# zhaodong-liu/GRAM

Hardware: AMD Instinct MI355X
Metric: users/sec @ beam=20 top-20 gen, Beauty T5-base; Recall@5 parity (higher is better)
Workload: dtype f16x3

## Files before the change

gram_amd/csrc/dec_attn.hip:

```cpp
#include <type_traits>

#include "common.h"
#include "prof.h"
#include "xattn_tile.h"

namespace {

__device__ __forceinline__ void xa_merge_w(float m0, float m1, float l0, float l1, float& w0, float& w1, float& inv) {
  const float M = fmaxf(fmaxf(GRAM_FMIN, m0), m1);
  w0 = __expf(m0 - M);
  w1 = __expf(m1 - M);
  inv = 1.f / __builtin_fmaf(l1, w1, l0 * w0);
}
__device__ __forceinline__ f32x4 xa_merge_o(f32x4 o0, f32x4 o1, float w0, float w1, float inv) {
  f32x4 r;
#pragma unroll
  for (int e = 0; e < 4; ++e) r[e] = __builtin_fmaf(o1[e], w1, o0[e] * w0) * inv;
  return r;
}

template <int NT, bool LIVE, int S, int NW>
__global__ __launch_bounds__(NW * 64) void cross_attn_kernel(
    const p16* __restrict__ q, const p16* __restrict__ kbank, const p16* __restrict__ vtbank,
    const uint8_t* __restrict__ mask, p16* __restrict__ out, int K, int H, int Sk, const int32_t* __restrict__ users,
    const int32_t* __restrict__ rowpos, long q_pstride, long bank_pstride, const uint32_t* __restrict__ key_bits) {
  using T = SplitTab<S>;
  constexpr int NB = NT * 16;
  static_assert(NW == 1 || NW == 2, "the merge is written for two waves");
  constexpr int PSTR = 2 * XA_TILE;
  constexpr int STAGE = S * PSTR;
  extern __shared__ __attribute__((aligned(16))) char smem[];
  float* sm_m = reinterpret_cast<float*>(smem);
  float* sm_l = sm_m + NW * NB;
  float* sm_o = sm_l + NW * NB;

  const int h = blockIdx.x, b = LIVE ? users[blockIdx.y] : blockIdx.y;
  const int tid = threadIdx.x, lane = tid & 63;
  const int wave = __builtin_amdgcn_readfirstlane(tid >> 6);
  const int c = lane & 15, g = lane >> 4;
  const int inner = H * 64;
  const char* kb = reinterpret_cast<const char*>(kbank + ((size_t)b * H + h) * Sk * 64);
  const char* vt = reinterpret_cast<const char*>(vtbank + ((size_t)b * H + h) * 64 * Sk);
  const uint8_t* mk = mask + (size_t)b * Sk;

  p16x8 qf[S][NT][2];
  f32x4 o[4][NT];
  float m[NT], l[NT];
#pragma unroll
  for (int nt = 0; nt < NT; ++nt) {
    m[nt] = GRAM_FMIN;
    l[nt] = 0.f;
#pragma unroll
    for (int mt = 0; mt < 4; ++mt) o[mt][nt] = (f32x4){0.f, 0.f, 0.f, 0.f};
  }

#pragma unroll
  for (int nt = 0; nt < NT; ++nt) {
    const int qrow = xa_row<LIVE>(b, K, 16 * nt + c, rowpos);
#pragma unroll
    for (int pc = 0; pc < S; ++pc)
#pragma unroll
      for (int kd = 0; kd < 2; ++kd)
        qf[pc][nt][kd] = qrow >= 0 ? ld_global_b128(q + pc * q_pstride + (size_t)qrow * inner + h * 64 + 32 * kd + 8 * g) : zero_bf16x8();
  }
  const int nsteps = Sk >> 5;
  uint32_t kb0 = 0, kb1 = 0;
  if (key_bits) {
    if (lane < nsteps) kb0 = key_bits[(size_t)b * 128 + lane];
    if (lane + 64 < nsteps) kb1 = key_bits[(size_t)b * 128 + 64 + lane];
  } else {
#pragma unroll
    for (int half = 0; half < 2; ++half) {
      const int st = lane + 64 * half;
      uint32_t bits = 0;
      if (st < nsteps) {
        const uint4* p = reinterpret_cast<const uint4*>(mk + 32 * st);
        const uint4 a = p[0], c2 = p[1];
        const uint32_t w8[8] = {a.x, a.y, a.z, a.w, c2.x, c2.y, c2.z, c2.w};
#pragma unroll
        for (int i = 0; i < 8; ++i)
#pragma unroll
          for (int j = 0; j < 4; ++j) bits |= ((w8[i] >> (8 * j)) & 0xffu) ? (1u << (4 * i + j)) : 0u;
      }
      if (half == 0) kb0 = bits; else kb1 = bits;
    }
  }
  unsigned long long v0 = __ballot(kb0 != 0u), v1 = __ballot(kb1 != 0u);
  if ((v0 | v1) == 0ull) {
    v0 = nsteps >= 64 ? ~0ull : ((1ull << nsteps) - 1ull);
    v1 = nsteps > 64 ? ((nsteps >= 128 ? ~0ull : ((1ull << (nsteps - 64)) - 1ull))) : 0ull;
  }
  v0 = __builtin_amdgcn_readfirstlane((unsigned)v0) | ((unsigned long long)__builtin_amdgcn_readfirstlane((unsigned)(v0 >> 32)) << 32);
  v1 = __builtin_amdgcn_readfirstlane((unsigned)v1) | ((unsigned long long)__builtin_amdgcn_readfirstlane((unsigned)(v1 >> 32)) << 32);
  int ord = 0;
  auto next = [&](int s) -> int {
    for (s = s + 1; s < nsteps; ++s) {
      const unsigned long long bit = (s < 64 ? (v0 >> s) : (v1 >> (s - 64))) & 1ull;
      if (bit) {
        const bool mine = ord == wave;
        ord = ord + 1 == NW ? 0 : ord + 1;
        if (mine) return s;
      }
    }
    return nsteps;
  };

  uint32_t koff[4], voff[4];
#pragma unroll
  for (int i = 0; i < 4; ++i) {
    const int kr = 8 * i + (lane >> 3);
    koff[i] = (uint32_t)(kr * 128 + (((lane & 7) ^ ksw(kr)) << 4));
    const int d = 16 * i + (lane >> 2);
    voff[i] = (uint32_t)(d * 64 + (((lane & 3) ^ vsw(d)) << 4));
  }
  const uint32_t stage0 = (uint32_t)(uintptr_t)(__attribute__((address_space(3))) char*)smem + wave * STAGE;
  auto issue_k = [&](int step) {
    const uint32_t dst = stage0;
#pragma unroll
    for (int pc = 0; pc < S; ++pc) {
      const char* kbase = kb + (size_t)pc * bank_pstride * 2 + (size_t)step * (32 * 128);
#pragma unroll
      for (int i = 0; i < 4; ++i) dma16_nt(dst + pc * PSTR + i * 1024, koff[i], kbase);
    }
  };
  auto issue_v = [&](int step) {
    const uint32_t dst = stage0;
#pragma unroll
    for (int pc = 0; pc < S; ++pc) {
      const char* vbase = vt + (size_t)pc * bank_pstride * 2 + (size_t)step * 4096;
#pragma unroll
      for (int i = 0; i < 4; ++i) dma16(dst + pc * PSTR + XA_TILE + i * 1024, voff[i], vbase);
    }
  };
  const int krow = 8 * (c >> 2) + (c & 3);
  p16x8 kf[S][2][2], vf[S][4];
  auto read_k = [&]() {
    const char* stg = smem + wave * STAGE;
#pragma unroll
    for (int pc = 0; pc < S; ++pc)
#pragma unroll
      for (int t = 0; t < 2; ++t)
#pragma unroll
        for (int kd = 0; kd < 2; ++kd) {
          const int r = krow + 4 * t;
          kf[pc][t][kd] = *reinterpret_cast<const p16x8*>(stg + pc * PSTR + r * 128 + (((g + 4 * kd) ^ ksw(r)) << 4));
        }
  };
  auto read_v = [&]() {
    const char* stg = smem + wave * STAGE;
#pragma unroll
    for (int pc = 0; pc < S; ++pc)
#pragma unroll
      for (int mt = 0; mt < 4; ++mt) {
        const int d = 16 * mt + c;
        vf[pc][mt] = *reinterpret_cast<const p16x8*>(stg + pc * PSTR + XA_TILE + d * 64 + ((g ^ vsw(d)) << 4));
      }
  };
  p16x8 pf[S][NT];
  auto math_qk = [&](int step) {
    const uint32_t kword = step < 64 ? (uint32_t)__builtin_amdgcn_readlane((int)kb0, step) : (uint32_t)__builtin_amdgcn_readlane((int)kb1, step - 64);
    const uint32_t kbits = kword >> (8 * g);
#pragma unroll
    for (int nt = 0; nt < NT; ++nt) {
      f32x4 s[2];
#pragma unroll
      for (int t = 0; t < 2; ++t) {
        f32x4 a = (f32x4){0.f, 0.f, 0.f, 0.f};
#pragma unroll
        for (int pr = 0; pr < T::NP; ++pr) {
          a = mfma16(kf[T::A[pr]][t][0], qf[T::B[pr]][nt][0], a);
          a = mfma16(kf[T::A[pr]][t][1], qf[T::B[pr]][nt][1], a);
        }
#pragma unroll
        for (int j = 0; j < 4; ++j) a[j] = ((kbits >> (4 * t + j)) & 1u) ? a[j] : GRAM_FMIN;
        s[t] = a;
      }
      float tm = fmaxf(fmaxf(fmaxf(s[0][0], s[0][1]), fmaxf(s[0][2], s[0][3])),
                       fmaxf(fmaxf(s[1][0], s[1][1]), fmaxf(s[1][2], s[1][3])));
      tm = fmaxf(tm, __shfl_xor(tm, 16, 64));
      tm = fmaxf(tm, __shfl_xor(tm, 32, 64));
      const float mn = fmaxf(m[nt], tm);
      const float alpha = __expf(m[nt] - mn);
      m[nt] = mn;
      float ps = 0.f;
#pragma unroll
      for (int t = 0; t < 2; ++t)
#pragma unroll
        for (int j = 0; j < 4; ++j) {
          float e = __expf(s[t][j] - mn);
          ps += e;
#pragma unroll
          for (int pc = 0; pc < S; ++pc) {
            const p16 eb = (p16)e;
            pf[pc][nt][4 * t + j] = eb;
            e -= (float)eb;
          }
        }
      l[nt] = xa_l_update(l[nt], alpha, ps);
#pragma unroll
      for (int mt = 0; mt < 4; ++mt) o[mt][nt] *= alpha;
    }
  };
  auto math_pv = [&]() {
#pragma unroll
    for (int mt = 0; mt < 4; ++mt)
#pragma unroll
      for (int nt = 0; nt < NT; ++nt)
#pragma unroll
        for (int pr = 0; pr < T::NP; ++pr) o[mt][nt] = mfma16(vf[T::A[pr]][mt], pf[T::B[pr]][nt], o[mt][nt]);
  };

  wait_vm<0>();
#pragma unroll
  for (int nt = 0; nt < NT; ++nt)
#pragma unroll
    for (int pc = 0; pc < S; ++pc)
#pragma unroll
      for (int kd = 0; kd < 2; ++kd) asm volatile("" : "+v"(qf[pc][nt][kd]));
  int cur = next(-1);
  if (cur < nsteps) {
    issue_k(cur);
    issue_v(cur);
  }
  while (cur < nsteps) {
    const int nxt = next(cur);
    wait_vm<4 * S>();
    read_k();
    if (nxt < nsteps) {
      asm volatile("s_waitcnt lgkmcnt(0)" ::: "memory");
      issue_k(nxt);
    }
    math_qk(cur);
    if (nxt < nsteps) wait_vm<4 * S>();
    else wait_vm<0>();
    read_v();
    if (nxt < nsteps) {
      asm volatile("s_waitcnt lgkmcnt(0)" ::: "memory");
      issue_v(nxt);
    }
    math_pv();
    cur = nxt;
  }

  if constexpr (NW == 1) {
#pragma unroll
    for (int nt = 0; nt < NT; ++nt) {
      float lt = l[nt];
      lt += __shfl_xor(lt, 16, 64);
      lt += __shfl_xor(lt, 32, 64);
      const float inv = 1.f / lt;
      const int orow = xa_row<LIVE>(b, K, 16 * nt + c, rowpos);
      if (orow >= 0) {
#pragma unroll
        for (int mt = 0; mt < 4; ++mt) xa_store<S>(out, orow, inner, h * 64 + 16 * mt + 4 * g, o[mt][nt] * inv);
      }
    }
    return;
  }
  gram_sync();
#pragma unroll
  for (int nt = 0; nt < NT; ++nt) {
    float lt = l[nt];
    lt += __shfl_xor(lt, 16, 64);
    lt += __shfl_xor(lt, 32, 64);
    const int beam = 16 * nt + c;
    if (g == 0) {
      sm_m[wave * NB + beam] = m[nt];
      sm_l[wave * NB + beam] = lt;
    }
#pragma unroll
    for (int mt = 0; mt < 4; ++mt)
      *reinterpret_cast<f32x4*>(sm_o + ((size_t)(wave * NB + beam)) * 64 + 16 * mt + 4 * g) = o[mt][nt];
  }
  gram_sync();
  for (int idx = tid; idx < K * 16; idx += NW * 64) {
    const int beam = idx >> 4, d4 = (idx & 15) * 4;
    float w0, w1, inv2;
    xa_merge_w(sm_m[beam], sm_m[NB + beam], sm_l[beam], sm_l[NB + beam], w0, w1, inv2);
    const f32x4 v = xa_merge_o(*reinterpret_cast<const f32x4*>(sm_o + ((size_t)beam) * 64 + d4),
                         *reinterpret_cast<const f32x4*>(sm_o + ((size_t)(NB + beam)) * 64 + d4), w0, w1, inv2);
    int orow = b * K + beam;
    if constexpr (LIVE) orow = rowpos[orow];
    if (orow >= 0) xa_store<S>(out, orow, inner, h * 64 + d4, v);
  }
}

constexpr int XA_RUN_MERGE = 4 * (4 * 64 * 16 + 2 * 64 * 4);
template <int S, int NW>
__global__ __launch_bounds__(2 * NW * 64, 2) void cross_attn_runs_kernel(
    const p16* __restrict__ q, const p16* __restrict__ kbank, const p16* __restrict__ vtbank, const uint8_t* __restrict__ mask,
    p16* __restrict__ out, int n_entries, int H, int Sk, const int32_t* __restrict__ ent_users, const int32_t* __restrict__ ent_rows,
    long q_pstride, long bank_pstride, const uint32_t* __restrict__ key_bits) {
  using T = SplitTab<S>;
  static_assert(NW == 1 || NW == 2, "the merge is written for two waves");
  constexpr int ER = GRAM_TAIL_ENTRY_ROWS;
  constexpr int MT = 4;
  static_assert(ER == 64, "a pair of entries is eight 16-row tiles");
  constexpr int PSTR = 2 * XA_TILE;
  constexpr int STAGE = S * PSTR;
  constexpr int MERGE = XA_RUN_MERGE;
  static_assert(MERGE == MT * (4 * 64 * 16 + 2 * 64 * 4), "O, m, l of up to MT tiles, one slot per lane");
  extern __shared__ __attribute__((aligned(16))) char smem[];

  const int h = blockIdx.x, lead = blockIdx.y;
  const int b = ent_users[lead];
  if (lead > 0 && ent_users[lead - 1] == b) return;
  int run_end = lead + 1;
  while (run_end < n_entries && ent_users[run_end] == b) ++run_end;

  const int tid = threadIdx.x, lane = tid & 63;
  const int wv = __builtin_amdgcn_readfirstlane(tid >> 6);
  const int wave = wv % NW, half = wv / NW;
  const int c = lane & 15, g = lane >> 4;
  const int inner = H * 64;
  const char* kb = reinterpret_cast<const char*>(kbank + ((size_t)b * H + h) * Sk * 64);
  const char* vt = reinterpret_cast<const char*>(vtbank + ((size_t)b * H + h) * 64 * Sk);
  const uint8_t* mk = mask + (size_t)b * Sk;

  const int nsteps = Sk >> 5;
  uint32_t kb0 = 0, kb1 = 0;
  if (key_bits) {
    if (lane < nsteps) kb0 = key_bits[(size_t)b * 128 + lane];
    if (lane + 64 < nsteps) kb1 = key_bits[(size_t)b * 128 + 64 + lane];
  } else {
#pragma unroll
    for (int hf = 0; hf < 2; ++hf) {
      const int st = lane + 64 * hf;
      uint32_t bits = 0;
      if (st < nsteps) {
        const uint4* p = reinterpret_cast<const uint4*>(mk + 32 * st);
        const uint4 a = p[0], c2 = p[1];
        const uint32_t w8[8] = {a.x, a.y, a.z, a.w, c2.x, c2.y, c2.z, c2.w};
#pragma unroll
        for (int i = 0; i < 8; ++i)
#pragma unroll
          for (int j = 0; j < 4; ++j) bits |= ((w8[i] >> (8 * j)) & 0xffu) ? (1u << (4 * i + j)) : 0u;
      }
      if (hf == 0) kb0 = bits; else kb1 = bits;
    }
  }
  unsigned long long v0 = __ballot(kb0 != 0u), v1 = __ballot(kb1 != 0u);
  if ((v0 | v1) == 0ull) {
    v0 = nsteps >= 64 ? ~0ull : ((1ull << nsteps) - 1ull);
    v1 = nsteps > 64 ? ((nsteps >= 128 ? ~0ull : ((1ull << (nsteps - 64)) - 1ull))) : 0ull;
  }
  v0 = __builtin_amdgcn_readfirstlane((unsigned)v0) | ((unsigned long long)__builtin_amdgcn_readfirstlane((unsigned)(v0 >> 32)) << 32);
  v1 = __builtin_amdgcn_readfirstlane((unsigned)v1) | ((unsigned long long)__builtin_amdgcn_readfirstlane((unsigned)(v1 >> 32)) << 32);
  int ord = 0;
  auto next = [&](int s) -> int {
    for (s = s + 1; s < nsteps; ++s) {
      const unsigned long long bit = (s < 64 ? (v0 >> s) : (v1 >> (s - 64))) & 1ull;
      if (bit) {
        const bool mine = ord == wave;
        ord = ord + 1 == NW ? 0 : ord + 1;
        if (mine) return s;
      }
    }
    return nsteps;
  };

  uint32_t koff[4], voff[4];
#pragma unroll
  for (int i = 0; i < 4; ++i) {
    const int kr = 8 * i + (lane >> 3);
    koff[i] = (uint32_t)(kr * 128 + (((lane & 7) ^ ksw(kr)) << 4));
    const int d = 16 * i + (lane >> 2);
    voff[i] = (uint32_t)(d * 64 + (((lane & 3) ^ vsw(d)) << 4));
  }
  const uint32_t stage0 = (uint32_t)(uintptr_t)(__attribute__((address_space(3))) char*)smem + wave * 2 * STAGE;
  const int nvalid = __popcll(v0) + __popcll(v1);
  const int trips = (nvalid + NW - 1) / NW;
  auto issue_k = [&](int step, int buf) {
    const uint32_t dst = stage0 + buf * STAGE;
#pragma unroll
    for (int pc = 0; pc < S; ++pc) {
      const char* kbase = kb + (size_t)pc * bank_pstride * 2 + (size_t)step * (32 * 128);
#pragma unroll
      for (int i = 0; i < 4; ++i) dma16_nt(dst + pc * PSTR + i * 1024, koff[i], kbase);
    }
  };
  auto issue_v = [&](int step, int buf) {
    const uint32_t dst = stage0 + buf * STAGE;
#pragma unroll
    for (int pc = 0; pc < S; ++pc) {
      const char* vbase = vt + (size_t)pc * bank_pstride * 2 + (size_t)step * 4096;
#pragma unroll
      for (int i = 0; i < 4; ++i) dma16(dst + pc * PSTR + XA_TILE + i * 1024, voff[i], vbase);
    }
  };
  const int krow = 8 * (c >> 2) + (c & 3);

  f32x4 o[4][MT];
  float m[MT], l[MT];
  auto sweep = [&](auto nl_c, const int32_t* __restrict__ rows, int tiles) __attribute__((always_inline)) {
    constexpr int NL = decltype(nl_c)::value;
    constexpr int NA = NL > 0 ? NL : 1;
    ord = 0;
    int cur = next(-1);
    if (cur < nsteps) {
      if (half == 0) issue_k(cur, 0);
      else issue_v(cur, 0);
    }
    p16x8 qf[S][NA][2];
#pragma unroll
    for (int nt = 0; nt < NL; ++nt) {
      const int qrow = rows[16 * ((tiles >> (4 * nt)) & 7) + c];
#pragma unroll
      for (int pc = 0; pc < S; ++pc)
#pragma unroll
        for (int kd = 0; kd < 2; ++kd)
          qf[pc][nt][kd] = qrow >= 0 ? ld_global_b128(q + pc * q_pstride + (size_t)qrow * inner + h * 64 + 32 * kd + 8 * g) : zero_bf16x8();
    }
    p16x8 kf[S][2][2], vf[S][4];
    auto read_k = [&](int buf) {
      const char* stg = smem + (wave * 2 + buf) * STAGE;
#pragma unroll
      for (int pc = 0; pc < S; ++pc)
#pragma unroll
        for (int t = 0; t < 2; ++t)
#pragma unroll
          for (int kd = 0; kd < 2; ++kd) {
            const int r = krow + 4 * t;
            kf[pc][t][kd] = *reinterpret_cast<const p16x8*>(stg + pc * PSTR + r * 128 + (((g + 4 * kd) ^ ksw(r)) << 4));
          }
    };
    auto read_v = [&](int buf) {
      const char* stg = smem + (wave * 2 + buf) * STAGE;
#pragma unroll
      for (int pc = 0; pc < S; ++pc)
#pragma unroll
        for (int mt = 0; mt < 4; ++mt) {
          const int d = 16 * mt + c;
          vf[pc][mt] = *reinterpret_cast<const p16x8*>(stg + pc * PSTR + XA_TILE + d * 64 + ((g ^ vsw(d)) << 4));
        }
    };
    p16x8 pf[S][NA];
    auto math_qk = [&](int step) {
      const uint32_t kword = step < 64 ? (uint32_t)__builtin_amdgcn_readlane((int)kb0, step) : (uint32_t)__builtin_amdgcn_readlane((int)kb1, step - 64);
      const uint32_t kbits = kword >> (8 * g);
#pragma unroll
      for (int nt = 0; nt < NL; ++nt) {
        f32x4 s[2];
#pragma unroll
        for (int t = 0; t < 2; ++t) {
          f32x4 a = (f32x4){0.f, 0.f, 0.f, 0.f};
#pragma unroll
          for (int pr = 0; pr < T::NP; ++pr) {
            a = mfma16(kf[T::A[pr]][t][0], qf[T::B[pr]][nt][0], a);
            a = mfma16(kf[T::A[pr]][t][1], qf[T::B[pr]][nt][1], a);
          }
#pragma unroll
          for (int j = 0; j < 4; ++j) a[j] = ((kbits >> (4 * t + j)) & 1u) ? a[j] : GRAM_FMIN;
          s[t] = a;
        }
        float tm = fmaxf(fmaxf(fmaxf(s[0][0], s[0][1]), fmaxf(s[0][2], s[0][3])),
                         fmaxf(fmaxf(s[1][0], s[1][1]), fmaxf(s[1][2], s[1][3])));
        tm = fmaxf(tm, __shfl_xor(tm, 16, 64));
        tm = fmaxf(tm, __shfl_xor(tm, 32, 64));
        const float mn = fmaxf(m[nt], tm);
        const float alpha = __expf(m[nt] - mn);
        m[nt] = mn;
        float ps = 0.f;
#pragma unroll
        for (int t = 0; t < 2; ++t)
#pragma unroll
          for (int j = 0; j < 4; ++j) {
            float e = __expf(s[t][j] - mn);
            ps += e;
#pragma unroll
            for (int pc = 0; pc < S; ++pc) {
              const p16 eb = (p16)e;
              pf[pc][nt][4 * t + j] = eb;
              e -= (float)eb;
            }
          }
        l[nt] = xa_l_update(l[nt], alpha, ps);
#pragma unroll
        for (int mt = 0; mt < 4; ++mt) o[mt][nt] *= alpha;
      }
    };
    auto math_pv = [&]() {
#pragma unroll
      for (int mt = 0; mt < 4; ++mt)
#pragma unroll
        for (int nt = 0; nt < NL; ++nt)
#pragma unroll
          for (int pr = 0; pr < T::NP; ++pr) o[mt][nt] = mfma16(vf[T::A[pr]][mt], pf[T::B[pr]][nt], o[mt][nt]);
    };
    wait_vm<0>();
#pragma unroll
    for (int nt = 0; nt < NL; ++nt)
#pragma unroll
      for (int pc = 0; pc < S; ++pc)
#pragma unroll
        for (int kd = 0; kd < 2; ++kd) asm volatile("" : "+v"(qf[pc][nt][kd]));
    for (int it = 0; it < trips; ++it) {
      const int buf = it & 1;
      wait_vm<0>();
      gram_sync();
      const int nxt = cur < nsteps ? next(cur) : nsteps;
      if (nxt < nsteps) {
        if (half == 0) issue_k(nxt, buf ^ 1);
        else issue_v(nxt, buf ^ 1);
      }
      if constexpr (NL > 0) {
        if (cur < nsteps) {
          read_k(buf);
          math_qk(cur);
          read_v(buf);
          math_pv();
        }
      }
      cur = nxt;
    }
  };

  for (int e0 = lead; e0 < run_end; e0 += 2) {
    const int32_t* rows = ent_rows + (size_t)e0 * ER;
    const int ntiles = e0 + 1 < run_end ? 2 * (ER / 16) : ER / 16;
    int nl = 0, tiles = 0, seen = 0;
#pragma unroll
    for (int t = 0; t < 2 * (ER / 16); ++t) {
      const int r = t < ntiles ? rows[16 * t + c] : -1;
      if (__ballot(r >= 0) != 0ull) {
        if ((seen & 1) == half) {
          tiles |= t << (4 * nl);
          ++nl;
        }
        ++seen;
      }
    }
    if (seen == 0) continue;
    nl = __builtin_amdgcn_readfirstlane(nl);
    tiles = __builtin_amdgcn_readfirstlane(tiles);
#pragma unroll
    for (int nt = 0; nt < MT; ++nt) {
      m[nt] = GRAM_FMIN;
      l[nt] = 0.f;
#pragma unroll
      for (int mt = 0; mt < 4; ++mt) o[mt][nt] = (f32x4){0.f, 0.f, 0.f, 0.f};
    }
    if (e0 != lead) gram_sync();
    switch (nl) {
      case 1: sweep(std::integral_constant<int, 1>{}, rows, tiles); break;
      case 2: sweep(std::integral_constant<int, 2>{}, rows, tiles); break;
      case 3: sweep(std::integral_constant<int, 3>{}, rows, tiles); break;
      case 4: sweep(std::integral_constant<int, 4>{}, rows, tiles); break;
      default: sweep(std::integral_constant<int, 0>{}, rows, tiles); break;
    }
    float* mg_o = reinterpret_cast<float*>(smem + half * MERGE);
    float* mg_m = mg_o + MT * 4 * 64 * 4;
    float* mg_l = mg_m + MT * 64;
    if constexpr (NW == 2) gram_sync();
#pragma unroll
    for (int nt = 0; nt < MT; ++nt) {
      if (nt < nl) {
        float lt = l[nt];
        lt += __shfl_xor(lt, 16, 64);
        lt += __shfl_xor(lt, 32, 64);
        l[nt] = lt;
        if constexpr (NW == 2) {
          if (wave == 1) {
            mg_m[nt * 64 + lane] = m[nt];
            mg_l[nt * 64 + lane] = lt;
#pragma unroll
            for (int mt = 0; mt < 4; ++mt) *reinterpret_cast<f32x4*>(mg_o + ((nt * 4 + mt) * 64 + lane) * 4) = o[mt][nt];
          }
        }
      }
    }
    if constexpr (NW == 2) gram_sync();
    if (wave == 0) {
#pragma unroll
      for (int nt = 0; nt < MT; ++nt) {
        if (nt < nl) {
          const int orow = rows[16 * ((tiles >> (4 * nt)) & 7) + c];
          if constexpr (NW == 2) {
            float w0, w1, inv2;
            xa_merge_w(m[nt], mg_m[nt * 64 + lane], l[nt], mg_l[nt * 64 + lane], w0, w1, inv2);
            if (orow >= 0) {
#pragma unroll
              for (int mt = 0; mt < 4; ++mt)
                xa_store<S>(out, orow, inner, h * 64 + 16 * mt + 4 * g,
                            xa_merge_o(o[mt][nt], *reinterpret_cast<const f32x4*>(mg_o + ((nt * 4 + mt) * 64 + lane) * 4), w0, w1, inv2));
            }
          } else {
            const float inv = 1.f / l[nt];
            if (orow >= 0) {
#pragma unroll
              for (int mt = 0; mt < 4; ++mt) xa_store<S>(out, orow, inner, h * 64 + 16 * mt + 4 * g, o[mt][nt] * inv);
            }
          }
        }
      }
    }
  }
}

struct XaLaunch {
  const void *q, *k, *vt;
  const uint8_t* mask;
  void* out;
  int B, K, H, Sk;
  const int32_t *users, *rowpos;
  long q_ps, bank_ps;
  const uint32_t* key_bits;
  hipStream_t st;
};

template <int NT, int S>
int launch_cross(const XaLaunch& a) {
  constexpr int NW = NT >= 3 ? 1 : 2;
  constexpr int NB = NT * 16;
  constexpr int stages = NW * S * 2 * XA_TILE, merge = NW == 1 ? 0 : (2 * NW * NB + NW * NB * 64) * 4;
  constexpr int smem = stages > merge ? stages : merge;
  static_assert(smem <= 160 * 1024, "the stages do not fit the LDS");
  static bool attr_set = false;
  if (!attr_set) {
    hipError_t e = hipFuncSetAttribute(reinterpret_cast<const void*>(cross_attn_kernel<NT, false, S, NW>),
                                       hipFuncAttributeMaxDynamicSharedMemorySize, smem);
    if (e == hipSuccess)
      e = hipFuncSetAttribute(reinterpret_cast<const void*>(cross_attn_kernel<NT, true, S, NW>),
                              hipFuncAttributeMaxDynamicSharedMemorySize, smem);
    if (e != hipSuccess) return (int)e;
    attr_set = true;
  }
  if (a.users)
    hipLaunchKernelGGL((cross_attn_kernel<NT, true, S, NW>), dim3(a.H, a.B), dim3(NW * 64), smem, a.st, (const p16*)a.q, (const p16*)a.k,
                       (const p16*)a.vt, a.mask, (p16*)a.out, a.K, a.H, a.Sk, a.users, a.rowpos, a.q_ps, a.bank_ps, a.key_bits);
  else
    hipLaunchKernelGGL((cross_attn_kernel<NT, false, S, NW>), dim3(a.H, a.B), dim3(NW * 64), smem, a.st, (const p16*)a.q, (const p16*)a.k,
                       (const p16*)a.vt, a.mask, (p16*)a.out, a.K, a.H, a.Sk, a.users, a.rowpos, a.q_ps, a.bank_ps, a.key_bits);
  GRAM_CHECK_LAUNCH();
  return 0;
}

template <int S>
int launch_cross_nt(const XaLaunch& a) {
  switch ((a.K + 15) / 16) {
    case 1: return launch_cross<1, S>(a);
    case 2: return launch_cross<2, S>(a);
    case 3: return launch_cross<3, S>(a);
    default: return launch_cross<4, S>(a);
  }
}

template <int S, int NW>
int launch_cross_entries(const XaLaunch& a) {
  constexpr int stages = NW * 2 * S * 2 * XA_TILE, merge = NW == 1 ? 0 : 2 * XA_RUN_MERGE;
  constexpr int smem = stages > merge ? stages : merge;
  static_assert(smem <= 160 * 1024, "the stages do not fit the LDS");
  static bool attr_set = false;
  if (!attr_set) {
    hipError_t e = hipFuncSetAttribute(reinterpret_cast<const void*>(cross_attn_runs_kernel<S, NW>),
                                       hipFuncAttributeMaxDynamicSharedMemorySize, smem);
    if (e != hipSuccess) return (int)e;
    attr_set = true;
  }
  hipLaunchKernelGGL((cross_attn_runs_kernel<S, NW>), dim3(a.H, a.B), dim3(2 * NW * 64), smem, a.st, (const p16*)a.q, (const p16*)a.k,
                     (const p16*)a.vt, a.mask, (p16*)a.out, a.B, a.H, a.Sk, a.users, a.rowpos, a.q_ps, a.bank_ps, a.key_bits);
  GRAM_CHECK_LAUNCH();
  return 0;
}

__global__ __launch_bounds__(128) void mask_key_bits_kernel(const uint8_t* __restrict__ mask, uint32_t* __restrict__ bits, int Sk) {
  const int b = blockIdx.x, st = threadIdx.x;
  uint32_t w = 0;
  if (st < (Sk >> 5)) {
    const uint4* p = reinterpret_cast<const uint4*>(mask + (size_t)b * Sk + 32 * st);
    const uint4 a = p[0], c2 = p[1];
    const uint32_t w8[8] = {a.x, a.y, a.z, a.w, c2.x, c2.y, c2.z, c2.w};
#pragma unroll
    for (int i = 0; i < 8; ++i)
#pragma unroll
      for (int j = 0; j < 4; ++j) w |= ((w8[i] >> (8 * j)) & 0xffu) ? (1u << (4 * i + j)) : 0u;
  }
  bits[(size_t)b * 128 + st] = w;
}

template <int S>
__global__ __launch_bounds__(256) void dec_self_attn_kernel(const p16* __restrict__ qkv, p16* __restrict__ kcache,
                                                            p16* __restrict__ vcache, const int32_t* __restrict__ anc,
                                                            const float* __restrict__ bias, p16* __restrict__ out, int R,
                                                            int H, int t, const int32_t* __restrict__ rows, long qkv_ps,
                                                            long cache_ps, const int32_t* __restrict__ qkv_rows) {
  const int rc = blockIdx.x, i = threadIdx.x;
  const int r = rows ? rows[rc] : rc;
  const int inner = H * 64, h = i >> 4;
  const p16* row = qkv + (size_t)(qkv_rows ? qkv_rows[rc] : rc) * 3 * inner + 4 * i;
  float qf[4] = {0.f, 0.f, 0.f, 0.f}, kn[4] = {0.f, 0.f, 0.f, 0.f}, vn[4] = {0.f, 0.f, 0.f, 0.f};
#pragma unroll
  for (int pc = S - 1; pc >= 0; --pc) {
    const p16x4 q4 = *reinterpret_cast<const p16x4*>(row + pc * qkv_ps);
    const p16x4 k4 = *reinterpret_cast<const p16x4*>(row + pc * qkv_ps + inner);
    const p16x4 v4 = *reinterpret_cast<const p16x4*>(row + pc * qkv_ps + 2 * inner);
    *reinterpret_cast<p16x4*>(kcache + pc * cache_ps + ((size_t)t * R + r) * inner + 4 * i) = k4;
    *reinterpret_cast<p16x4*>(vcache + pc * cache_ps + ((size_t)t * R + r) * inner + 4 * i) = v4;
#pragma unroll
    for (int e = 0; e < 4; ++e) {
      qf[e] += (float)q4[e];
      kn[e] += (float)k4[e];
      vn[e] += (float)v4[e];
    }
  }
  float m = -INFINITY, l = 0.f, acc[4] = {0.f, 0.f, 0.f, 0.f};
  auto attend = [&](int j, const float (&kj)[4], const float (&vj)[4]) {
    float s = qf[0] * kj[0] + qf[1] * kj[1] + qf[2] * kj[2] + qf[3] * kj[3];
    s += __shfl_xor(s, 1, 64);
    s += __shfl_xor(s, 2, 64);
    s += __shfl_xor(s, 4, 64);
    s += __shfl_xor(s, 8, 64);
    s += bias[h * GRAM_MAX_DEC_LEN + (t - j)];
    const float mn = fmaxf(m, s);
    const float alpha = __expf(m - mn);
    const float p = __expf(s - mn);
    m = mn;
    l = l * alpha + p;
#pragma unroll
    for (int e = 0; e < 4; ++e) acc[e] = acc[e] * alpha + p * vj[e];
  };
  constexpr int U = 8;
  for (int j0 = 0; j0 < t; j0 += U) {
    int a[U];
#pragma unroll
    for (int u = 0; u < U; ++u) a[u] = anc[(size_t)min(j0 + u, t - 1) * R + r];
    p16x4 kk[U][S], vv[U][S];
#pragma unroll
    for (int u = 0; u < U; ++u) {
      const size_t off = ((size_t)min(j0 + u, t - 1) * R + a[u]) * inner + 4 * i;
#pragma unroll
      for (int pc = 0; pc < S; ++pc) {
        kk[u][pc] = ld_stream_b64(kcache + pc * cache_ps + off);
        vv[u][pc] = ld_stream_b64(vcache + pc * cache_ps + off);
      }
    }
#pragma unroll
    for (int u = 0; u < U; ++u) {
      if (j0 + u < t) {
        float kj[4] = {0.f, 0.f, 0.f, 0.f}, vj[4] = {0.f, 0.f, 0.f, 0.f};
#pragma unroll
        for (int pc = S - 1; pc >= 0; --pc)
#pragma unroll
          for (int e = 0; e < 4; ++e) {
            kj[e] += (float)kk[u][pc][e];
            vj[e] += (float)vv[u][pc][e];
          }
        attend(j0 + u, kj, vj);
      }
    }
  }
  attend(t, kn, vn);
  const float inv = 1.f / l;
#pragma unroll
  for (int e = 0; e < 4; ++e) acc[e] *= inv;
#pragma unroll
  for (int pc = 0; pc < S; ++pc) {
    p16x4 o;
#pragma unroll
    for (int e = 0; e < 4; ++e) {
      o[e] = (p16)acc[e];
      acc[e] -= (float)o[e];
    }
    *reinterpret_cast<p16x4*>(out + (size_t)rc * inner * S + (S == 2 ? inter_off(4 * i, pc) : 4 * i)) = o;
  }
}

}

extern "C" int gram_cross_attn_entries_split(const void* q, const void* k_layer, const void* vt_layer, const uint8_t* mask, void* out,
                                             int n_entries, int K, int H, int S, const int32_t* ent_users, const int32_t* ent_rows,
                                             int pieces, int64_t q_pstride, int64_t bank_pstride, const uint32_t* key_bits,
                                             void* stream) {
  if (!q || !out || !ent_users || !ent_rows || n_entries < 1 || K < 1 || K > GRAM_MAX_BEAMS || H < 1 || S < 32 || (S & 31) ||
      S > 4096 || pieces < 1 || pieces > GRAM_MAX_PIECES)
    return GRAM_E_ARG;
  if (pieces > 1 && (q_pstride < 1 || bank_pstride < (int64_t)H * S * 64)) return GRAM_E_ARG;
  if ((reinterpret_cast<uintptr_t>(mask) & 15) || (reinterpret_cast<uintptr_t>(k_layer) & 15) || (reinterpret_cast<uintptr_t>(vt_layer) & 15))
    return GRAM_E_ARG;
  hipStream_t st = (hipStream_t)stream;
  gram_prof::Scope prof(GRAM_K_CROSS_ATTN, st, 4.0 * n_entries * H * S * 64 * pieces);
  const XaLaunch a{q, k_layer, vt_layer, mask, out, n_entries, GRAM_TAIL_ENTRY_ROWS, H, S, ent_users, ent_rows, (long)q_pstride,
                   (long)bank_pstride, key_bits, st};
  const bool one_wave = (K + 15) / 16 >= 3;
  if (pieces == 2) return one_wave ? launch_cross_entries<2, 1>(a) : launch_cross_entries<2, 2>(a);
  return one_wave ? launch_cross_entries<1, 1>(a) : launch_cross_entries<1, 2>(a);
}

extern "C" int gram_mask_key_bits(const uint8_t* mask, uint32_t* key_bits, int B, int S, void* stream) {
  if (!mask || !key_bits || B < 1 || S < 32 || (S & 31) || S > 4096 || (reinterpret_cast<uintptr_t>(mask) & 15)) return GRAM_E_ARG;
  hipLaunchKernelGGL(mask_key_bits_kernel, dim3(B), dim3(128), 0, (hipStream_t)stream, mask, key_bits, S);
  GRAM_CHECK_LAUNCH();
  return 0;
}

extern "C" int gram_cross_attn_decode_split(const void* q, const void* k_layer, const void* vt_layer, const uint8_t* mask, void* out,
                                            int B, int K, int H, int S, const int32_t* users, const int32_t* rowpos, int pieces,
                                            int64_t q_pstride, int64_t bank_pstride, const uint32_t* key_bits, void* stream) {
  if (B < 1 || K < 1 || K > GRAM_MAX_BEAMS || H < 1 || S < 32 || (S & 31) || S > 4096 || pieces < 1 || pieces > GRAM_MAX_PIECES ||
      (users == nullptr) != (rowpos == nullptr))
    return GRAM_E_ARG;
  if (pieces > 1 && (q_pstride < 1 || bank_pstride < (int64_t)H * S * 64)) return GRAM_E_ARG;
  if ((reinterpret_cast<uintptr_t>(mask) & 15) || (reinterpret_cast<uintptr_t>(k_layer) & 15) || (reinterpret_cast<uintptr_t>(vt_layer) & 15))
    return GRAM_E_ARG;
  hipStream_t st = (hipStream_t)stream;
  gram_prof::Scope prof(GRAM_K_CROSS_ATTN, st, 4.0 * B * H * S * 64 * pieces);
  const XaLaunch a{q, k_layer, vt_layer, mask, out, B, K, H, S, users, rowpos, (long)q_pstride, (long)bank_pstride, key_bits, st};
  return pieces == 2 ? launch_cross_nt<2>(a) : launch_cross_nt<1>(a);
}

extern "C" int gram_cross_attn_decode(const void* q, const void* k_layer, const void* vt_layer, const uint8_t* mask, void* out,
                                      int B, int K, int H, int S, void* stream) {
  return gram_cross_attn_decode_split(q, k_layer, vt_layer, mask, out, B, K, H, S, nullptr, nullptr, 1, 0, 0, nullptr, stream);
}

extern "C" int gram_cross_attn_decode_live(const void* q, const void* k_layer, const void* vt_layer, const uint8_t* mask, void* out,
                                           int n_users, const int32_t* users, const int32_t* rowpos, int K, int H, int S,
                                           void* stream) {
  if (!users || !rowpos) return GRAM_E_ARG;
  return gram_cross_attn_decode_split(q, k_layer, vt_layer, mask, out, n_users, K, H, S, users, rowpos, 1, 0, 0, nullptr, stream);
}

extern "C" int gram_dec_self_attn_split(const void* qkv, void* kcache, void* vcache, const int32_t* anc, const float* bias, void* out,
                                        int R, int n_rows, const int32_t* rows, int H, int t, int Tmax, int pieces,
                                        int64_t qkv_pstride, int64_t cache_pstride, void* stream) {
  return gram_dec_self_attn_rows_split(qkv, nullptr, kcache, vcache, anc, bias, out, R, n_rows, rows, H, t, Tmax, pieces, qkv_pstride,
                                       cache_pstride, stream);
}

extern "C" int gram_dec_self_attn_rows_split(const void* qkv, const int32_t* qkv_rows, void* kcache, void* vcache, const int32_t* anc,
                                             const float* bias, void* out, int R, int n_rows, const int32_t* rows, int H, int t,
                                             int Tmax, int pieces, int64_t qkv_pstride, int64_t cache_pstride, void* stream) {
  if (R < 1 || n_rows < 1 || n_rows > R || H < 1 || H > 16 || t < 0 || t >= Tmax || Tmax > GRAM_MAX_DEC_LEN || pieces < 1 ||
      pieces > GRAM_MAX_PIECES)
    return GRAM_E_ARG;
  if (pieces > 1 && (qkv_pstride < 1 || cache_pstride < (int64_t)Tmax * R * H * 64)) return GRAM_E_ARG;
  hipStream_t st = (hipStream_t)stream;
  gram_prof::Scope prof(GRAM_K_DEC_SELF_ATTN, st, 4.0 * n_rows * H * 64 * (t + 1) * pieces);
  const dim3 grid(n_rows), block(H * 16);
  if (pieces == 2)
    hipLaunchKernelGGL(dec_self_attn_kernel<2>, grid, block, 0, st, (const p16*)qkv, (p16*)kcache, (p16*)vcache, anc, bias,
                       (p16*)out, R, H, t, rows, (long)qkv_pstride, (long)cache_pstride, qkv_rows);
  else
    hipLaunchKernelGGL(dec_self_attn_kernel<1>, grid, block, 0, st, (const p16*)qkv, (p16*)kcache, (p16*)vcache, anc, bias,
                       (p16*)out, R, H, t, rows, (long)qkv_pstride, (long)cache_pstride, qkv_rows);
  GRAM_CHECK_LAUNCH();
  return 0;
}

extern "C" int gram_dec_self_attn(const void* qkv, void* kcache, void* vcache, const int32_t* anc, const float* bias, void* out,
                                  int R, int H, int t, int Tmax, void* stream) {
  return gram_dec_self_attn_split(qkv, kcache, vcache, anc, bias, out, R, R, nullptr, H, t, Tmax, 1, 0, 0, stream);
}

extern "C" int gram_dec_self_attn_live(const void* qkv, void* kcache, void* vcache, const int32_t* anc, const float* bias,
                                       void* out, int R, int n_rows, const int32_t* rows, int H, int t, int Tmax, void* stream) {
  if (!rows) return GRAM_E_ARG;
  return gram_dec_self_attn_split(qkv, kcache, vcache, anc, bias, out, R, n_rows, rows, H, t, Tmax, 1, 0, 0, stream);
}
```

Before: 3292.

## Split cross-attention run kernel across four wave parts with shared K/V DMA ring

The runs kernel now launches four parts of NW waves instead of two. Each part owns at most two of the eight 16-row query tiles, and the four parts split one step's K and V DMA instructions between them into a shared ring. The kernel also finds the run of entries with one ballot across a lane window instead of a serial scan, prefetches the first entry's rows, and interleaves K/V LDS reads with the MFMAs in smaller chunks to lower register pressure, aiming for more occupancy and more in-flight work per head. In exchange the block is larger, merge LDS grows with WP, and every step needs a barrier across more waves.

Result: no change. 3302 (median of 6 runs) (+0.3%).

```diff
diff --git a/gram_amd/csrc/dec_attn.hip b/gram_amd/csrc/dec_attn.hip
--- a/gram_amd/csrc/dec_attn.hip
+++ b/gram_amd/csrc/dec_attn.hip
@@ -285,32 +285,45 @@
   }
 }
 
-constexpr int XA_RUN_MERGE = 4 * (4 * 64 * 16 + 2 * 64 * 4);
+constexpr int XA_RUN_WP = 4;
+constexpr int XA_RUN_MERGE = 2 * (4 * 64 * 16 + 2 * 64 * 4);
 template <int S, int NW>
-__global__ __launch_bounds__(2 * NW * 64, 2) void cross_attn_runs_kernel(
+__global__ __launch_bounds__(XA_RUN_WP * NW * 64, 4) void cross_attn_runs_kernel(
     const p16* __restrict__ q, const p16* __restrict__ kbank, const p16* __restrict__ vtbank, const uint8_t* __restrict__ mask,
     p16* __restrict__ out, int n_entries, int H, int Sk, const int32_t* __restrict__ ent_users, const int32_t* __restrict__ ent_rows,
     long q_pstride, long bank_pstride, const uint32_t* __restrict__ key_bits) {
   using T = SplitTab<S>;
   static_assert(NW == 1 || NW == 2, "the merge is written for two waves");
   constexpr int ER = GRAM_TAIL_ENTRY_ROWS;
-  constexpr int MT = 4;
-  static_assert(ER == 64, "a pair of entries is eight 16-row tiles");
-  constexpr int PSTR = 2 * XA_TILE;
-  constexpr int STAGE = S * PSTR;
+  constexpr int WP = XA_RUN_WP;
+  constexpr int MT = 2;
+  static_assert(ER == 64 && WP * MT == 8, "a pair of entries is eight 16-row tiles");
+  static_assert(S == 1 || S == 2, "a step's 8 S DMA instructions are dealt to four waves");
+  constexpr int KT = S * XA_TILE;
+  constexpr int RING = 4 * KT;
   constexpr int MERGE = XA_RUN_MERGE;
   static_assert(MERGE == MT * (4 * 64 * 16 + 2 * 64 * 4), "O, m, l of up to MT tiles, one slot per lane");
   extern __shared__ __attribute__((aligned(16))) char smem[];
 
   const int h = blockIdx.x, lead = blockIdx.y;
-  const int b = ent_users[lead];
-  if (lead > 0 && ent_users[lead - 1] == b) return;
-  int run_end = lead + 1;
-  while (run_end < n_entries && ent_users[run_end] == b) ++run_end;
-
   const int tid = threadIdx.x, lane = tid & 63;
+  const int eidx = lead - 1 + lane;
+  const bool e_ok = eidx >= 0 && eidx < n_entries;
+  const int eu = e_ok ? ent_users[eidx] : 0;
+  int rows0[2 * (GRAM_TAIL_ENTRY_ROWS / 16)];
+#pragma unroll
+  for (int t = 0; t < 2 * (GRAM_TAIL_ENTRY_ROWS / 16); ++t)
+    rows0[t] = (t < GRAM_TAIL_ENTRY_ROWS / 16 || lead + 1 < n_entries) ? ent_rows[(size_t)lead * GRAM_TAIL_ENTRY_ROWS + 16 * t + (lane & 15)] : -1;
+  const int b = __builtin_amdgcn_readlane(eu, 1);
+  const unsigned long long same = __ballot(e_ok && eu == b);
+  if (same & 1ull) return;
+  const int run_len = __builtin_ctzll(~(same >> 1));
+  int run_end = lead + run_len;
+  if (run_len == 63)
+    while (run_end < n_entries && ent_users[run_end] == b) ++run_end;
+
   const int wv = __builtin_amdgcn_readfirstlane(tid >> 6);
-  const int wave = wv % NW, half = wv / NW;
+  const int wave = wv % NW, part = wv / NW;
   const int c = lane & 15, g = lane >> 4;
   const int inner = H * 64;
   const char* kb = reinterpret_cast<const char*>(kbank + ((size_t)b * H + h) * Sk * 64);
@@ -339,13 +352,16 @@
       if (hf == 0) kb0 = bits; else kb1 = bits;
     }
   }
-  unsigned long long v0 = __ballot(kb0 != 0u), v1 = __ballot(kb1 != 0u);
-  if ((v0 | v1) == 0ull) {
-    v0 = nsteps >= 64 ? ~0ull : ((1ull << nsteps) - 1ull);
-    v1 = nsteps > 64 ? ((nsteps >= 128 ? ~0ull : ((1ull << (nsteps - 64)) - 1ull))) : 0ull;
-  }
-  v0 = __builtin_amdgcn_readfirstlane((unsigned)v0) | ((unsigned long long)__builtin_amdgcn_readfirstlane((unsigned)(v0 >> 32)) << 32);
-  v1 = __builtin_amdgcn_readfirstlane((unsigned)v1) | ((unsigned long long)__builtin_amdgcn_readfirstlane((unsigned)(v1 >> 32)) << 32);
+  unsigned long long v0 = 0ull, v1 = 0ull;
+  auto valid_steps = [&]() {
+    v0 = __ballot(kb0 != 0u), v1 = __ballot(kb1 != 0u);
+    if ((v0 | v1) == 0ull) {
+      v0 = nsteps >= 64 ? ~0ull : ((1ull << nsteps) - 1ull);
+      v1 = nsteps > 64 ? ((nsteps >= 128 ? ~0ull : ((1ull << (nsteps - 64)) - 1ull))) : 0ull;
+    }
+    v0 = __builtin_amdgcn_readfirstlane((unsigned)v0) | ((unsigned long long)__builtin_amdgcn_readfirstlane((unsigned)(v0 >> 32)) << 32);
+    v1 = __builtin_amdgcn_readfirstlane((unsigned)v1) | ((unsigned long long)__builtin_amdgcn_readfirstlane((unsigned)(v1 >> 32)) << 32);
+  };
   int ord = 0;
   auto next = [&](int s) -> int {
     for (s = s + 1; s < nsteps; ++s) {
@@ -359,100 +375,88 @@
     return nsteps;
   };
 
-  uint32_t koff[4], voff[4];
-#pragma unroll
-  for (int i = 0; i < 4; ++i) {
+  constexpr int ND = 2 * S;
+  const bool dma_v = part >= WP / 2;
+  const int dma_pc = (ND * (part & 1)) >> 2, dma_i0 = (ND * (part & 1)) & 3;
+  uint32_t doff[ND];
+#pragma unroll
+  for (int j = 0; j < ND; ++j) {
+    const int i = dma_i0 + j;
     const int kr = 8 * i + (lane >> 3);
-    koff[i] = (uint32_t)(kr * 128 + (((lane & 7) ^ ksw(kr)) << 4));
     const int d = 16 * i + (lane >> 2);
-    voff[i] = (uint32_t)(d * 64 + (((lane & 3) ^ vsw(d)) << 4));
-  }
-  const uint32_t stage0 = (uint32_t)(uintptr_t)(__attribute__((address_space(3))) char*)smem + wave * 2 * STAGE;
-  const int nvalid = __popcll(v0) + __popcll(v1);
-  const int trips = (nvalid + NW - 1) / NW;
-  auto issue_k = [&](int step, int buf) {
-    const uint32_t dst = stage0 + buf * STAGE;
-#pragma unroll
-    for (int pc = 0; pc < S; ++pc) {
-      const char* kbase = kb + (size_t)pc * bank_pstride * 2 + (size_t)step * (32 * 128);
-#pragma unroll
-      for (int i = 0; i < 4; ++i) dma16_nt(dst + pc * PSTR + i * 1024, koff[i], kbase);
-    }
-  };
-  auto issue_v = [&](int step, int buf) {
-    const uint32_t dst = stage0 + buf * STAGE;
-#pragma unroll
-    for (int pc = 0; pc < S; ++pc) {
-      const char* vbase = vt + (size_t)pc * bank_pstride * 2 + (size_t)step * 4096;
-#pragma unroll
-      for (int i = 0; i < 4; ++i) dma16(dst + pc * PSTR + XA_TILE + i * 1024, voff[i], vbase);
+    doff[j] = dma_v ? (uint32_t)(d * 64 + (((lane & 3) ^ vsw(d)) << 4)) : (uint32_t)(kr * 128 + (((lane & 7) ^ ksw(kr)) << 4));
+  }
+  const char* dma_src = (dma_v ? vt : kb) + (size_t)dma_pc * bank_pstride * 2;
+  const uint32_t ring0 = (uint32_t)(uintptr_t)(__attribute__((address_space(3))) char*)smem + wave * RING;
+  const uint32_t dma_dst = ring0 + (dma_v ? 2 * KT : 0) + dma_pc * XA_TILE + dma_i0 * 1024;
+  auto issue = [&](int step, int buf) {
+    const uint32_t dst = dma_dst + buf * KT;
+    const char* base = dma_src + (size_t)step * 4096;
+    if (dma_v) {
+#pragma unroll
+      for (int j = 0; j < ND; ++j) dma16(dst + j * 1024, doff[j], base);
+    } else {
+#pragma unroll
+      for (int j = 0; j < ND; ++j) dma16_nt(dst + j * 1024, doff[j], base);
     }
   };
   const int krow = 8 * (c >> 2) + (c & 3);
 
   f32x4 o[4][MT];
   float m[MT], l[MT];
-  auto sweep = [&](auto nl_c, const int32_t* __restrict__ rows, int tiles) __attribute__((always_inline)) {
+  int trow[MT];
+  auto sweep = [&](auto nl_c) __attribute__((always_inline)) {
     constexpr int NL = decltype(nl_c)::value;
     constexpr int NA = NL > 0 ? NL : 1;
+    p16x8 qf[S][NA][2];
+    int gq = g;
+    asm volatile("" : "+v"(gq));
+#pragma unroll
+    for (int nt = 0; nt < NL; ++nt) {
+      const int qrow = trow[nt];
+#pragma unroll
+      for (int pc = 0; pc < S; ++pc)
+#pragma unroll
+        for (int kd = 0; kd < 2; ++kd)
+          qf[pc][nt][kd] = qrow >= 0 ? ld_global_b128(q + pc * q_pstride + (size_t)qrow * inner + h * 64 + 32 * kd + 8 * gq) : zero_bf16x8();
+    }
+    valid_steps();
+    const int trips = (__popcll(v0) + __popcll(v1) + NW - 1) / NW;
     ord = 0;
     int cur = next(-1);
-    if (cur < nsteps) {
-      if (half == 0) issue_k(cur, 0);
-      else issue_v(cur, 0);
-    }
-    p16x8 qf[S][NA][2];
-#pragma unroll
-    for (int nt = 0; nt < NL; ++nt) {
-      const int qrow = rows[16 * ((tiles >> (4 * nt)) & 7) + c];
-#pragma unroll
-      for (int pc = 0; pc < S; ++pc)
-#pragma unroll
-        for (int kd = 0; kd < 2; ++kd)
-          qf[pc][nt][kd] = qrow >= 0 ? ld_global_b128(q + pc * q_pstride + (size_t)qrow * inner + h * 64 + 32 * kd + 8 * g) : zero_bf16x8();
-    }
-    p16x8 kf[S][2][2], vf[S][4];
-    auto read_k = [&](int buf) {
-      const char* stg = smem + (wave * 2 + buf) * STAGE;
-#pragma unroll
-      for (int pc = 0; pc < S; ++pc)
-#pragma unroll
-        for (int t = 0; t < 2; ++t)
-#pragma unroll
-          for (int kd = 0; kd < 2; ++kd) {
-            const int r = krow + 4 * t;
-            kf[pc][t][kd] = *reinterpret_cast<const p16x8*>(stg + pc * PSTR + r * 128 + (((g + 4 * kd) ^ ksw(r)) << 4));
-          }
-    };
-    auto read_v = [&](int buf) {
-      const char* stg = smem + (wave * 2 + buf) * STAGE;
-#pragma unroll
-      for (int pc = 0; pc < S; ++pc)
-#pragma unroll
-        for (int mt = 0; mt < 4; ++mt) {
-          const int d = 16 * mt + c;
-          vf[pc][mt] = *reinterpret_cast<const p16x8*>(stg + pc * PSTR + XA_TILE + d * 64 + ((g ^ vsw(d)) << 4));
-        }
-    };
+    if (cur < nsteps) issue(cur, 0);
     p16x8 pf[S][NA];
-    auto math_qk = [&](int step) {
+    auto math_qk = [&](int step, int buf) {
+      const char* stg = smem + wave * RING + buf * KT;
       const uint32_t kword = step < 64 ? (uint32_t)__builtin_amdgcn_readlane((int)kb0, step) : (uint32_t)__builtin_amdgcn_readlane((int)kb1, step - 64);
       const uint32_t kbits = kword >> (8 * g);
+      f32x4 sa[NA][2];
+#pragma unroll
+      for (int t = 0; t < 2; ++t) {
+        p16x8 kf[S][2];
+        const int r = krow + 4 * t;
+#pragma unroll
+        for (int pc = 0; pc < S; ++pc)
+#pragma unroll
+          for (int kd = 0; kd < 2; ++kd)
+            kf[pc][kd] = *reinterpret_cast<const p16x8*>(stg + pc * XA_TILE + r * 128 + (((g + 4 * kd) ^ ksw(r)) << 4));
+#pragma unroll
+        for (int nt = 0; nt < NL; ++nt) {
+          f32x4 a = (f32x4){0.f, 0.f, 0.f, 0.f};
+#pragma unroll
+          for (int pr = 0; pr < T::NP; ++pr) {
+            a = mfma16(kf[T::A[pr]][0], qf[T::B[pr]][nt][0], a);
+            a = mfma16(kf[T::A[pr]][1], qf[T::B[pr]][nt][1], a);
+          }
+#pragma unroll
+          for (int j = 0; j < 4; ++j) a[j] = ((kbits >> (4 * t + j)) & 1u) ? a[j] : GRAM_FMIN;
+          sa[nt][t] = a;
+        }
+        __builtin_amdgcn_sched_barrier(0);
+      }
 #pragma unroll
       for (int nt = 0; nt < NL; ++nt) {
-        f32x4 s[2];
-#pragma unroll
-        for (int t = 0; t < 2; ++t) {
-          f32x4 a = (f32x4){0.f, 0.f, 0.f, 0.f};
-#pragma unroll
-          for (int pr = 0; pr < T::NP; ++pr) {
-            a = mfma16(kf[T::A[pr]][t][0], qf[T::B[pr]][nt][0], a);
-            a = mfma16(kf[T::A[pr]][t][1], qf[T::B[pr]][nt][1], a);
-          }
-#pragma unroll
-          for (int j = 0; j < 4; ++j) a[j] = ((kbits >> (4 * t + j)) & 1u) ? a[j] : GRAM_FMIN;
-          s[t] = a;
-        }
+        const f32x4 (&s)[2] = sa[nt];
         float tm = fmaxf(fmaxf(fmaxf(s[0][0], s[0][1]), fmaxf(s[0][2], s[0][3])),
                          fmaxf(fmaxf(s[1][0], s[1][1]), fmaxf(s[1][2], s[1][3])));
         tm = fmaxf(tm, __shfl_xor(tm, 16, 64));
@@ -479,13 +483,26 @@
         for (int mt = 0; mt < 4; ++mt) o[mt][nt] *= alpha;
       }
     };
-    auto math_pv = [&]() {
-#pragma unroll
-      for (int mt = 0; mt < 4; ++mt)
-#pragma unroll
-        for (int nt = 0; nt < NL; ++nt)
-#pragma unroll
-          for (int pr = 0; pr < T::NP; ++pr) o[mt][nt] = mfma16(vf[T::A[pr]][mt], pf[T::B[pr]][nt], o[mt][nt]);
+    auto math_pv = [&](int buf) {
+      const char* stg = smem + wave * RING + (2 + buf) * KT;
+#pragma unroll
+      for (int m2 = 0; m2 < 4; m2 += 2) {
+        p16x8 vf[S][2];
+#pragma unroll
+        for (int pc = 0; pc < S; ++pc)
+#pragma unroll
+          for (int i = 0; i < 2; ++i) {
+            const int d = 16 * (m2 + i) + c;
+            vf[pc][i] = *reinterpret_cast<const p16x8*>(stg + pc * XA_TILE + d * 64 + ((g ^ vsw(d)) << 4));
+          }
+#pragma unroll
+        for (int i = 0; i < 2; ++i)
+#pragma unroll
+          for (int nt = 0; nt < NL; ++nt)
+#pragma unroll
+            for (int pr = 0; pr < T::NP; ++pr) o[m2 + i][nt] = mfma16(vf[T::A[pr]][i], pf[T::B[pr]][nt], o[m2 + i][nt]);
+        __builtin_amdgcn_sched_barrier(0);
+      }
     };
     wait_vm<0>();
 #pragma unroll
@@ -499,37 +516,41 @@
       wait_vm<0>();
       gram_sync();
       const int nxt = cur < nsteps ? next(cur) : nsteps;
-      if (nxt < nsteps) {
-        if (half == 0) issue_k(nxt, buf ^ 1);
-        else issue_v(nxt, buf ^ 1);
-      }
+      if (nxt < nsteps) issue(nxt, buf ^ 1);
       if constexpr (NL > 0) {
         if (cur < nsteps) {
-          read_k(buf);
-          math_qk(cur);
-          read_v(buf);
-          math_pv();
+          math_qk(cur, buf);
+          math_pv(buf);
         }
       }
       cur = nxt;
     }
   };
 
-  for (int e0 = lead; e0 < run_end; e0 += 2) {
-    const int32_t* rows = ent_rows + (size_t)e0 * ER;
-    const int ntiles = e0 + 1 < run_end ? 2 * (ER / 16) : ER / 16;
-    int nl = 0, tiles = 0, seen = 0;
+  int nl = 0, tiles = 0, seen = 0;
+  auto census = [&](int ntiles, auto slot) __attribute__((always_inline)) {
+    nl = 0, tiles = 0, seen = 0;
+    trow[0] = trow[1] = -1;
 #pragma unroll
     for (int t = 0; t < 2 * (ER / 16); ++t) {
-      const int r = t < ntiles ? rows[16 * t + c] : -1;
+      const int r = t < ntiles ? slot(t) : -1;
       if (__ballot(r >= 0) != 0ull) {
-        if ((seen & 1) == half) {
+        if ((seen & (WP - 1)) == part) {
+          if (nl == 0) trow[0] = r;
+          else trow[1] = r;
           tiles |= t << (4 * nl);
           ++nl;
         }
         ++seen;
       }
     }
+  };
+  census(lead + 1 < run_end ? 2 * (ER / 16) : ER / 16, [&](int t) { return rows0[t]; });
+  for (int e0 = lead; e0 < run_end; e0 += 2) {
+    if (e0 != lead) {
+      const int32_t* rows = ent_rows + (size_t)e0 * ER;
+      census(e0 + 1 < run_end ? 2 * (ER / 16) : ER / 16, [&](int t) { return rows[16 * t + c]; });
+    }
     if (seen == 0) continue;
     nl = __builtin_amdgcn_readfirstlane(nl);
     tiles = __builtin_amdgcn_readfirstlane(tiles);
@@ -542,13 +563,14 @@
     }
     if (e0 != lead) gram_sync();
     switch (nl) {
-      case 1: sweep(std::integral_constant<int, 1>{}, rows, tiles); break;
-      case 2: sweep(std::integral_constant<int, 2>{}, rows, tiles); break;
-      case 3: sweep(std::integral_constant<int, 3>{}, rows, tiles); break;
-      case 4: sweep(std::integral_constant<int, 4>{}, rows, tiles); break;
-      default: sweep(std::integral_constant<int, 0>{}, rows, tiles); break;
-    }
-    float* mg_o = reinterpret_cast<float*>(smem + half * MERGE);
+      case 1: sweep(std::integral_constant<int, 1>{}); break;
+      case 2: sweep(std::integral_constant<int, 2>{}); break;
+      default: sweep(std::integral_constant<int, 0>{}); break;
+    }
+    int orow_of[MT];
+#pragma unroll
+    for (int nt = 0; nt < MT; ++nt) orow_of[nt] = nt < nl ? ent_rows[(size_t)e0 * ER + 16 * ((tiles >> (4 * nt)) & 7) + c] : -1;
+    float* mg_o = reinterpret_cast<float*>(smem + part * MERGE);
     float* mg_m = mg_o + MT * 4 * 64 * 4;
     float* mg_l = mg_m + MT * 64;
     if constexpr (NW == 2) gram_sync();
@@ -571,24 +593,26 @@
     }
     if constexpr (NW == 2) gram_sync();
     if (wave == 0) {
+      int gs = g;
+      asm volatile("" : "+v"(gs));
 #pragma unroll
       for (int nt = 0; nt < MT; ++nt) {
         if (nt < nl) {
-          const int orow = rows[16 * ((tiles >> (4 * nt)) & 7) + c];
+          const int orow = orow_of[nt];
           if constexpr (NW == 2) {
             float w0, w1, inv2;
             xa_merge_w(m[nt], mg_m[nt * 64 + lane], l[nt], mg_l[nt * 64 + lane], w0, w1, inv2);
             if (orow >= 0) {
 #pragma unroll
               for (int mt = 0; mt < 4; ++mt)
-                xa_store<S>(out, orow, inner, h * 64 + 16 * mt + 4 * g,
+                xa_store<S>(out, orow, inner, h * 64 + 16 * mt + 4 * gs,
                             xa_merge_o(o[mt][nt], *reinterpret_cast<const f32x4*>(mg_o + ((nt * 4 + mt) * 64 + lane) * 4), w0, w1, inv2));
             }
           } else {
             const float inv = 1.f / l[nt];
             if (orow >= 0) {
 #pragma unroll
-              for (int mt = 0; mt < 4; ++mt) xa_store<S>(out, orow, inner, h * 64 + 16 * mt + 4 * g, o[mt][nt] * inv);
+              for (int mt = 0; mt < 4; ++mt) xa_store<S>(out, orow, inner, h * 64 + 16 * mt + 4 * gs, o[mt][nt] * inv);
             }
           }
         }
@@ -647,7 +671,7 @@
 
 template <int S, int NW>
 int launch_cross_entries(const XaLaunch& a) {
-  constexpr int stages = NW * 2 * S * 2 * XA_TILE, merge = NW == 1 ? 0 : 2 * XA_RUN_MERGE;
+  constexpr int stages = NW * 2 * S * 2 * XA_TILE, merge = NW == 1 ? 0 : XA_RUN_WP * XA_RUN_MERGE;
   constexpr int smem = stages > merge ? stages : merge;
   static_assert(smem <= 160 * 1024, "the stages do not fit the LDS");
   static bool attr_set = false;
@@ -657,7 +681,7 @@
     if (e != hipSuccess) return (int)e;
     attr_set = true;
   }
-  hipLaunchKernelGGL((cross_attn_runs_kernel<S, NW>), dim3(a.H, a.B), dim3(2 * NW * 64), smem, a.st, (const p16*)a.q, (const p16*)a.k,
+  hipLaunchKernelGGL((cross_attn_runs_kernel<S, NW>), dim3(a.H, a.B), dim3(XA_RUN_WP * NW * 64), smem, a.st, (const p16*)a.q, (const p16*)a.k,
                      (const p16*)a.vt, a.mask, (p16*)a.out, a.B, a.H, a.Sk, a.users, a.rowpos, a.q_ps, a.bank_ps, a.key_bits);
   GRAM_CHECK_LAUNCH();
   return 0;
```
